# danieldugas/DeepMimic_mujoco

Measured on AMD Instinct MI355X. Metric: env-steps/sec (whole node), 34-DoF humanoid, 4096 envs, at 1/2/4/8 MI355X, higher is better.
Workload: dtype f32

## Files before the change

deepmimic_mujoco_amd/csrc/dm_abi.hip:

```cpp
#include "../../include/deepmimic_hip.h"
#include "dm_device.h"
#include "dm_topology.h"

#include <math.h>
#include <stdio.h>
#include <string.h>

#include <string>
#include <vector>

#include "dm_kernels.hip"
#include "dm_ppo.hip"
#include "dm_policy.hip"
#include "dm_ppo_mlp.hip"
#include "dm_ppo_wide.hip"
#include "dm_sac.hip"

struct DmEngine {
  DmConfig cfg;
  DmModel model;
  int N = 0;
  DmDev *dT = nullptr;
  float *dState = nullptr;
  float *dArScratch = nullptr;
  float *dClipRows[DM_MAX_CLIPS] = {nullptr};
  float *dClipReset[DM_MAX_CLIPS] = {nullptr};
  int clipL[DM_MAX_CLIPS] = {0};
  int clipFlags[DM_MAX_CLIPS] = {0};
  float *debug = nullptr;
  int32_t *dOrder = nullptr;
  int32_t *dCost = nullptr;
  static constexpr int NEV = 512;
  hipEvent_t ev0[NEV] = {}, ev1[NEV] = {};
  long nrec = 0;
  long nlaunch = 0;
  int stride = 1;
  int waves = 0;
  bool timing = false;
  float last_ms = 0;
  std::string err;
};

static int fail(DmEngine *e, int code, const char *what, hipError_t he = hipSuccess) {
  if (e) {
    e->err = what;
    if (he != hipSuccess) { e->err += ": "; e->err += hipGetErrorString(he); }
  }
  return code;
}
#define HIPCHK(e, call)                                   \
  do {                                                    \
    hipError_t _r = (call);                               \
    if (_r != hipSuccess) return fail(e, DM_EHIP, #call, _r); \
  } while (0)

extern "C" void dm_default_config(DmConfig *c) {
  memset(c, 0, sizeof(*c));
  c->num_envs = 1;
  c->max_ep_length = 1000;
  c->vel_obs_scale = 0.1f;
  c->low_z = 0.7f;
  c->high_z = 2.0f;
  c->w_pose = 0.75f; c->w_vel = 0.1f; c->w_end_eff = 0.15f; c->w_com = 0.0f; c->w_joint_limit = -0.1f;
  c->obs_bound = 100.0f;
  c->seed = 1234;
  c->auto_reset = 1;
  c->device = 0;
  c->lpt_schedule = 1;
  c->task = DM_TASK_DPENV;
  c->amnesty_steps = 150;
// ... 99 lines not shown
static int check_model(DmEngine *e, const DmModel &m) {
  if (m.nq != DM_NQ || m.nv != DM_NV || m.nu != DM_NU || m.nbody != DM_NBODY || m.ngeom != DM_NGEOM)
    return fail(e, DM_EINVAL, "model dimensions do not match the compiled-in humanoid3d dimensions");
  if (m.integrator != DM_INT_RK4 && m.integrator != DM_INT_EULER) return fail(e, DM_EINVAL, "integrator must be RK4 or Euler");
  if (m.npair < 0 || m.npair > DM_MAXPAIR) return fail(e, DM_EINVAL, "npair out of range");
  for (int b = 1; b < DM_NBODY; b++) {
    if (m.body_quat[b][0] != 1.0) return fail(e, DM_EINVAL, "kernels assume identity body quaternions");
    if (m.body_dofnum[b] != 1 && m.body_dofnum[b] != 3 && m.body_dofnum[b] != 6)
      return fail(e, DM_EINVAL, "kernels assume 1- or 3-hinge bodies under a free root");
    if (m.body_depth[b] < 1 || m.body_depth[b] > 4) return fail(e, DM_EINVAL, "tree depth > 4");
  }
  for (int j = 0; j < DM_NJNT; j++)
    for (int i = 0; i < 3; i++)
      if (m.jnt_pos[j][i] != 0.0) return fail(e, DM_EINVAL, "kernels assume joint anchors at the body origin");
  if (m.jnt_type[0] != DM_JNT_FREE || m.jnt_body[0] != 1) return fail(e, DM_EINVAL, "joint 0 must be the free root");
  for (int k = 0; k < DM_NV; k++)
    if (m.dof_parent[k] != topo::PARENT[k] || m.dof_Madr[k] != topo::MADR[k])
      return fail(e, DM_EINVAL, "dof tree differs from the compiled-in topology (regenerate csrc/dm_topology.h)");
  for (int b = 0; b < DM_NBODY; b++)
    if (m.body_parent[b] != topo::BPARENT[b])
      return fail(e, DM_EINVAL, "body tree differs from the compiled-in topology (regenerate csrc/dm_topology.h)");
  return DM_OK;
}

extern "C" int dm_create(const DmModel *model, const DmConfig *cfg, DmHandle *out) {
  if (!model || !cfg || !out || cfg->num_envs < 1) return DM_EINVAL;
  int ndev = 0;
  if (hipGetDeviceCount(&ndev) != hipSuccess || ndev <= 0) return DM_ENODEV;
  DmEngine *e = new DmEngine();
  e->cfg = *cfg;
  e->model = *model;
  e->N = cfg->num_envs;
  if (const char *w = getenv("DM_WAVES")) e->waves = atoi(w);
  int rc = check_model(e, *model);
  if (rc != DM_OK) { fprintf(stderr, "dm_create: %s\n", e->err.c_str()); delete e; return rc; }
  if (hipSetDevice(cfg->device) != hipSuccess) { delete e; return DM_ENODEV; }
  DmDev T;
  build_tables(*model, T);
  if (hipMalloc(&e->dT, sizeof(DmDev)) != hipSuccess) { delete e; return DM_ENOMEM; }
  hipMemcpy(e->dT, &T, sizeof(DmDev), hipMemcpyHostToDevice);
  size_t sb = (size_t)e->N * DMK_STATE_STRIDE * sizeof(float);
  if (hipMalloc(&e->dState, sb) != hipSuccess) { hipFree(e->dT); delete e; return DM_ENOMEM; }
  std::vector<float> init((size_t)e->N * DMK_STATE_STRIDE, 0.f);
  for (int i = 0; i < e->N; i++)
    for (int k = 0; k < DM_NQ; k++) init[(size_t)i * DMK_STATE_STRIDE + DMS_QPOS + k] = (float)model->qpos0[k];
  hipMemcpy(e->dState, init.data(), sb, hipMemcpyHostToDevice);
  if (hipMalloc(&e->dArScratch, (size_t)e->N * DMK_MAXROW * DMK_MAXROW * sizeof(float)) != hipSuccess) {
    hipFree(e->dState); hipFree(e->dT); delete e; return DM_ENOMEM;
  }
  if (hipMalloc(&e->dOrder, e->N * sizeof(int32_t)) != hipSuccess || hipMalloc(&e->dCost, e->N * sizeof(int32_t)) != hipSuccess) {
    hipFree(e->dArScratch); hipFree(e->dState); hipFree(e->dT); delete e; return DM_ENOMEM;
  }
  hipMemset(e->dCost, 0, e->N * sizeof(int32_t));
  { std::vector<int32_t> ident(e->N);
    for (int i = 0; i < e->N; i++) ident[i] = i;
    hipMemcpy(e->dOrder, ident.data(), e->N * sizeof(int32_t), hipMemcpyHostToDevice); }
  for (int i = 0; i < DmEngine::NEV; i++) { hipEventCreate(&e->ev0[i]); hipEventCreate(&e->ev1[i]); }
  *out = e;
  return DM_OK;
}

extern "C" int dm_destroy(DmHandle e) {
  if (!e) return DM_EINVAL;
  hipSetDevice(e->cfg.device);
  hipDeviceSynchronize();
  for (int i = 0; i < DM_MAX_CLIPS; i++) { if (e->dClipRows[i]) hipFree(e->dClipRows[i]); if (e->dClipReset[i]) hipFree(e->dClipReset[i]); }
// ... 87 lines not shown
  HIPCHK(e, hipSetDevice(e->cfg.device));
  hipLaunchKernelGGL(dm_get_clip_kernel, dim3((e->N + 255) / 256), dim3(256), 0, (hipStream_t)stream, e->dState, clip_ids, e->N);
  HIPCHK(e, hipGetLastError());
  return DM_OK;
}

extern "C" int dm_set_clip_flags(DmHandle e, int clip_id, int flags) {
  if (!e || clip_id < 0 || clip_id >= DM_MAX_CLIPS) return DM_EINVAL;
  e->clipFlags[clip_id] = flags;
  return DM_OK;
}

extern "C" int dm_set_env_clips(DmHandle e, const int32_t *clip_ids, void *stream) {
  if (!e) return DM_EINVAL;
  HIPCHK(e, hipSetDevice(e->cfg.device));
  hipLaunchKernelGGL(dm_set_clip_kernel, dim3((e->N + 255) / 256), dim3(256), 0, (hipStream_t)stream, e->dState, clip_ids, e->N);
  HIPCHK(e, hipGetLastError());
  return DM_OK;
}

static void fill_launch(DmEngine *e, DmLaunch &P, int mode) {
  memset(&P, 0, sizeof(P));
  P.T = e->dT;
  P.state = e->dState;
  P.ar_scratch = e->dArScratch;
  for (int i = 0; i < DM_MAX_CLIPS; i++) { P.clips[i].rows = e->dClipRows[i]; P.clips[i].reset = e->dClipReset[i]; P.clips[i].L = e->clipL[i]; P.clips[i].flags = e->clipFlags[i]; }
  P.N = e->N; P.mode = mode; P.auto_reset = e->cfg.auto_reset; P.max_ep_length = e->cfg.max_ep_length;
  P.vel_obs_scale = e->cfg.vel_obs_scale; P.low_z = e->cfg.low_z; P.high_z = e->cfg.high_z; P.obs_bound = e->cfg.obs_bound;
  P.w_pose = e->cfg.w_pose; P.w_vel = e->cfg.w_vel; P.w_ee = e->cfg.w_end_eff; P.w_com = e->cfg.w_com; P.w_jl = e->cfg.w_joint_limit;
  P.seed = e->cfg.seed;
  P.amnesty_steps = e->cfg.amnesty_steps; P.to_getup_len = e->cfg.to_getup_len;
  P.integrator = e->cfg.integrator == DM_CFG_INT_EULER ? DM_INT_EULER : e->cfg.integrator == DM_CFG_INT_RK4 ? DM_INT_RK4 : e->model.integrator;
  P.f8 = e->cfg.stale_contact_slots ? 1 : 0;
  P.debug = e->debug;
}

static int launch(DmEngine *e, DmLaunch &P, int nslots, void *stream) {
  P.nslots = nslots;
  if (e->clipL[0] < 1) return fail(e, DM_EINVAL, "no clip loaded (dm_load_clip clip 0 first)");
  if (e->cfg.task == DM_TASK_COMBINED && (e->clipL[1] < 1 || e->clipL[2] < 2))
    return fail(e, DM_EINVAL, "combined task needs clips 0,1,2 = walk, run, getup");
  HIPCHK(e, hipSetDevice(e->cfg.device));
  hipStream_t s = (hipStream_t)stream;
  const int evi = (int)(e->nrec % DmEngine::NEV);
  const bool rec = e->timing && (e->nlaunch++ % e->stride) == 0;
  if (rec) hipEventRecord(e->ev0[evi], s);
  const dim3 grid((P.nslots + DMK_ENVS_PER_BLOCK - 1) / DMK_ENVS_PER_BLOCK), block(64 * DMK_ENVS_PER_BLOCK);
  const bool three_waves = e->waves == 3 || (e->waves == 0 && P.nslots >= 3072);
  if (e->cfg.task == DM_TASK_COMBINED) {
    if (three_waves) hipLaunchKernelGGL(dm_step_combined_kernel_w3, grid, block, 0, s, P);
    else hipLaunchKernelGGL(dm_step_combined_kernel, grid, block, 0, s, P);
#ifdef DM_EXPERIMENT_W4
  } else if (e->waves == 4) {
    hipLaunchKernelGGL(dm_step_kernel_w4, grid, block, 0, s, P);
#endif
  } else if (three_waves) {
    hipLaunchKernelGGL(dm_step_kernel_w3, grid, block, 0, s, P);
  } else {
    hipLaunchKernelGGL(dm_step_kernel, grid, block, 0, s, P);
  }
  if (rec) { hipEventRecord(e->ev1[evi], s); e->nrec++; }
  HIPCHK(e, hipGetLastError());
  return DM_OK;
}

extern "C" int dm_reset(DmHandle e, const uint8_t *mask, const int32_t *idx_init, float *obs_out, void *stream) {
// ... 172 lines not shown
```

deepmimic_mujoco_amd/csrc/dm_device.h:

```cpp
#pragma once

#include <hip/hip_runtime.h>
#include <stdint.h>

#include "../../include/dm_model.h"

#define DMK_NQ DM_NQ
#define DMK_NV DM_NV
#define DMK_NU DM_NU
#define DMK_NB DM_NBODY
#define DMK_NG DM_NGEOM
#define DMK_MAXCON DM_MAXCON
#define DMK_MAXROW DM_MAXROW
#define DMK_LANEROW 64
#define DMK_REGROW 32
#define DMK_MSTRIDE 35
#define DMK_MAXANC 12
#define DMK_STATE_STRIDE 144
#define DMK_CLIP_ROW 80

struct DmPairDev {
  int16_t g1, g2;
  int8_t t1, t2, pad0, pad1;
  float margin, rbsum;
// ... 75 lines not shown
};

#define DMS_QPOS 0
#define DMS_QVEL 35
#define DMS_WARM 69
#define DMS_CTRL 103
#define DMS_IDX 131
#define DMS_EPLEN 132
#define DMS_EPREW 133
#define DMS_CLIP 134
#define DMS_RCNT 135
#define DMS_F8R 136
#define DMS_F8L 137

#define DMK_RESET_ROW 72

struct DmClipDev {
  const float *rows;
  const float *reset;
  int32_t L, flags;
};

enum { DMK_MODE_STEP = 0, DMK_MODE_FORCED = 1, DMK_MODE_RESET = 2, DMK_MODE_SETSTATE = 3,
       DMK_MODE_PHYSICS = 4 };

struct DmLaunch {
  const DmDev *T;
  float *state;
  float *ar_scratch;
  DmClipDev clips[8];
  int32_t N, nslots, mode, auto_reset, max_ep_length;
  int32_t amnesty_steps, to_getup_len;
  int32_t integrator, f8;
  float vel_obs_scale, low_z, high_z, obs_bound;
  float w_pose, w_vel, w_ee, w_com, w_jl;
  uint64_t seed;
  const float *actions;
  const float *in_qpos;
  const float *in_qvel;
  const float *in_warm;
  const float *in_ctrl;
  const int32_t *env_ids;
  int32_t *cost;
  const uint8_t *mask;
  const int32_t *idx_init;
  int32_t run_forward;
  float *obs, *rew, *terms, *terminal_obs, *debug;
  uint8_t *done;
  int32_t *reason;
};
```

deepmimic_mujoco_amd/csrc/dm_kernels.hip:

```cpp
#include "../../include/deepmimic_hip.h"
#include "dm_device.h"
#include "dm_topology.h"

#include <math.h>

#include <type_traits>

#define SYNC()                                              \
  do {                                                      \
    __builtin_amdgcn_fence(__ATOMIC_RELEASE, "wavefront");  \
    __builtin_amdgcn_wave_barrier();                        \
    __builtin_amdgcn_fence(__ATOMIC_ACQUIRE, "wavefront");  \
  } while (0)
#define DMK_ENVS_PER_BLOCK 1
#ifndef DMK_WAVES_PER_SIMD
#define DMK_WAVES_PER_SIMD 2
#endif
#ifdef DM_PROFILE
#define PROF_DECL do { if ((threadIdx.x & 63) == 0) { for (int _i = 0; _i < 16; _i++) g_S.prof[_i] = 0; for (int _i = 0; _i < 4; _i++) g_S.prof_stage[_i] = 0; g_S.prof_t = g_S.prof_t0 = __builtin_amdgcn_s_memtime(); } } while (0)
#define PROF_STAGE(i) do { if ((threadIdx.x & 63) == 0 && (i) < 4) g_S.prof_stage[i] = (unsigned)(__builtin_amdgcn_s_memtime() - g_S.prof_t0); } while (0)
#define PROF(i) do { if ((threadIdx.x & 63) == 0) { unsigned long long _t = __builtin_amdgcn_s_memtime(); g_S.prof[i] += (unsigned)(_t - g_S.prof_t); g_S.prof_t = _t; } } while (0)
#if DM_PROFILE == 2
#define PROF2(i) PROF(i)
#else
// ... 52 lines not shown
  }
};
__device__ __forceinline__ float solve_LT(float x, const float dv, const int negdep, const float *M) {
  StaticFor<0, DMK_NV - 1>::run([&](auto ic) {
    constexpr int i = DMK_NV - 1 - decltype(ic)::value;
    const float xi = rl(x * dv, i);
    const float l = lane_sel<topo::anc_mask(i)>(M[topo::MADR[i] + topo::NANC[i] + negdep], 0.f);
    x = fmaf(-l, xi, x);
    return true;
  });
  return x;
}
__device__ __forceinline__ float solve_L(float x, const float dv, const int mrow, const float *M) {
  StaticFor<0, DMK_NV - 1>::run([&](auto jc) {
    constexpr int j = decltype(jc)::value;
    const float xj = rl(x * dv, j);
    const float l = lane_sel<topo::desc_mask(j)>(M[mrow - topo::NANC[j]], 0.f);
    x = fmaf(-l, xj, x);
    return true;
  });
  return x;
}
template <int CTRL>
__device__ __forceinline__ float dpp_mov(float v) {
  return __int_as_float(__builtin_amdgcn_update_dpp(0, __float_as_int(v), CTRL, 0xF, 0xF, true));
}
__device__ __forceinline__ float wave_sum(float v) {
  v += dpp_mov<0xB1>(v);
  v += dpp_mov<0x4E>(v);
  v += dpp_mov<0x141>(v);
  v += dpp_mov<0x140>(v);
  return (rl(v, 0) + rl(v, 16)) + (rl(v, 32) + rl(v, 48));
}
__device__ __forceinline__ unsigned long long lanemask_lt(int lane) {
  return (lane == 0) ? 0ull : (~0ull >> (64 - lane));
}
__device__ __forceinline__ int prefix_count(bool flag, int lane, int *total) {
  unsigned long long m = __ballot(flag);
  *total = __popcll(m);
  return __popcll(m & lanemask_lt(lane));
}

__device__ __forceinline__ void cross3(float *r, const float *a, const float *b) {
  float x = a[1] * b[2] - a[2] * b[1], y = a[2] * b[0] - a[0] * b[2], z = a[0] * b[1] - a[1] * b[0];
  r[0] = x; r[1] = y; r[2] = z;
}
__device__ __forceinline__ float dot3(const float *a, const float *b) {
  return a[0] * b[0] + a[1] * b[1] + a[2] * b[2];
}
__device__ __forceinline__ void quat_mul(float *r, const float *a, const float *b) {
  float w = a[0] * b[0] - a[1] * b[1] - a[2] * b[2] - a[3] * b[3];
  float x = a[0] * b[1] + a[1] * b[0] + a[2] * b[3] - a[3] * b[2];
  float y = a[0] * b[2] - a[1] * b[3] + a[2] * b[0] + a[3] * b[1];
  float z = a[0] * b[3] + a[1] * b[2] - a[2] * b[1] + a[3] * b[0];
  r[0] = w; r[1] = x; r[2] = y; r[3] = z;
}
__device__ __forceinline__ void quat_rot(float *r, const float *q, const float *v) {
  float t[3], u[3];
  cross3(t, q + 1, v);
  t[0] *= 2.f; t[1] *= 2.f; t[2] *= 2.f;
  cross3(u, q + 1, t);
  r[0] = v[0] + q[0] * t[0] + u[0];
  r[1] = v[1] + q[0] * t[1] + u[1];
  r[2] = v[2] + q[0] * t[2] + u[2];
}
__device__ __forceinline__ void quat2mat(float *m, const float *q) {
// ... 888 lines not shown
      int cnt = __popc(c.valid);
      unsigned long long lt = lanemask_lt(lane);
      unsigned long long b0 = __ballot(cnt & 1), b1 = __ballot(cnt & 2), b2 = __ballot(cnt & 4);
      int off = __popcll(b0 & lt) + 2 * __popcll(b1 & lt) + 4 * __popcll(b2 & lt);
      int total = __popcll(b0) + 2 * __popcll(b1) + 4 * __popcll(b2);
      if (total == 0) continue;
      int w = base + off;
#pragma unroll
      for (int s = 0; s < 4; s++) {
        if ((c.valid >> s) & 1) {
          if (w < DMK_MAXCON) {
            float fr[9] = {c.n[s][0], c.n[s][1], c.n[s][2], c.t[0], c.t[1], c.t[2], 0, 0, 0};
            make_frame(fr);
            S.c_dist[w] = c.d[s];
            for (int q = 0; q < 3; q++) S.c_pos[w][q] = c.p[s][q];
            for (int q = 0; q < 9; q++) S.c_frame[w][q] = fr[q];
            S.c_g1[w] = g1; S.c_g2[w] = g2;
          }
          w++;
        }
      }
      base += total;
    }
    if (base > DMK_MAXCON) { overflow |= 1; base = DMK_MAXCON; }
    ncon = base;
    SYNC();

    PROF(5);
  return ncon | (overflow << 8);
}

template <bool MF>
__device__ __forceinline__ void build_row(GDev &T, EnvLds &S, const int r, const int nefc, const float (&com)[3],
                                          float (&J)[DMK_NV], float &R, float &Dd, float &aref, float &bb, float &jw) {
      float rpos = 0, rmargin = 0, rdiag = 1, mu = 0;
      int rtype = -1, full = 0;
      float wl[3] = {0, 0, 0}, wa[3] = {0, 0, 0};
      unsigned long long cm1 = 0, cm2 = 0;
      int ldof = -1;
      float lsign = 0;
      if (r < nefc) {
        int info = S.rowinfo[r];
        if (info < 0) {
          int v = -info - 1;
          ldof = v >> 1;
          lsign = (v & 1) ? -1.f : 1.f;
          rtype = 0;
          float q = S.qpos[ldof + 1];
          rpos = (v & 1) ? (T.d_hi[ldof] - q) : (q - T.d_lo[ldof]);
          rmargin = 0;
          rdiag = T.d_invw[ldof];
        } else {
          int ci = (info >> 3) & 0x3F, e = info & 7;
          full = (info & 0x4000) ? 1 : 0;
          int g1 = S.c_g1[ci], g2 = S.c_g2[ci];
          int b1 = T.g_body[g1], b2 = T.g_body[g2];
          int cd1 = T.g_condim[g1], cd2 = T.g_condim[g2];
          int dim = cd1 > cd2 ? cd1 : cd2;
          mu = fmaxf(T.g_mu[g1], T.g_mu[g2]);
          float fr[9];
          for (int i = 0; i < 9; i++) fr[i] = S.c_frame[ci][i];
          float tran = T.b_invw[b1] + T.b_invw[b2];
          if (dim < 3) {
            rtype = 1;
            wl[0] = fr[0]; wl[1] = fr[1]; wl[2] = fr[2];
            rdiag = tran;
          } else {
            rtype = 2;
            const bool second = (e >> 1) != 0;
            const float tx = second ? fr[6] : fr[3], ty = second ? fr[7] : fr[4], tz = second ? fr[8] : fr[5];
            float sg = (e & 1) ? -mu : mu;
            wl[0] = fr[0] + sg * tx; wl[1] = fr[1] + sg * ty; wl[2] = fr[2] + sg * tz;
            rdiag = tran + mu * mu * tran;
          }
          float off[3] = {S.c_pos[ci][0] - com[0], S.c_pos[ci][1] - com[1], S.c_pos[ci][2] - com[2]};
          cross3(wa, off, wl);
          cm1 = T.b_chain[b1]; cm2 = T.b_chain[b2];
          rpos = S.c_dist[ci];
          rmargin = fmaxf(T.g_margin[g1], T.g_margin[g2]);
        }
      }
      float vel = 0, jqs = 0;
      jw = 0;
      float vals[32];
      if (MF) {
        const float wv[6] = {wa[0], wa[1], wa[2], wl[0], wl[1], wl[2]};
        const int lane_ = (int)(threadIdx.x & 63);
        const float *cdp = &S.cdof[lane_ & 31][lane_ >> 5];
        mfma_f16v acc;
#pragma unroll
        for (int v = 0; v < 16; v++) acc[v] = 0.f;
#pragma unroll
        for (int p = 0; p < 3; p++) {
          const auto sw = __builtin_amdgcn_permlane32_swap(__float_as_uint(wv[2 * p]), __float_as_uint(wv[2 * p + 1]), false, false);
          acc = __builtin_amdgcn_mfma_f32_32x32x2f32(cdp[2 * p], __uint_as_float(sw[0]), acc, 0, 0, 0);
        }
#pragma unroll
        for (int v = 0; v < 16; v++) {
          const auto sw = __builtin_amdgcn_permlane32_swap(__float_as_uint(acc[v]), __float_as_uint(acc[v]), false, false);
          vals[(v / 4) * 8 + (v % 4)] = acc[v];
          vals[(v / 4) * 8 + (v % 4) + 4] = __uint_as_float(sw[1]);
        }
      }
#pragma unroll
      for (int k = 0; k < DMK_NV; k++) {
        float val;
        if (MF && k < 32) {
          val = vals[k];
        } else {
          const float4 ca = *reinterpret_cast<const float4 *>(&S.cdof[k][0]);
          const float2 cb = *reinterpret_cast<const float2 *>(&S.cdof[k][4]);
          val = ca.x * wa[0] + ca.y * wa[1] + ca.z * wa[2] + ca.w * wl[0] + cb.x * wl[1] + cb.y * wl[2];
        }
        float sg = (float)((int)((cm2 >> k) & 1ull) - (int)((cm1 >> k) & 1ull));
        float j = (k == ldof) ? lsign : sg * val;
        J[k] = j;
        vel += j * S.qvel[k];
        jqs += j * S.qacc_smooth[k];
        jw += j * S.warm[k];
      }
      R = 1; Dd = 0; aref = 0; bb = 0;
      if (r < nefc) {
        float sol[5] = {T.solimp[0], T.solimp[1], T.solimp[2], T.solimp[3], T.solimp[4]};
        float imp = impedance(sol, rpos, rmargin);
        R = fmaxf(MINVALF, (1 - imp) * rdiag / imp);
        if (rtype == 2 && full) R = 2 * mu * mu * R;
        aref = -T.B * vel - T.K * imp * (rpos - rmargin);
        bb = jqs - aref;
        Dd = 1.0f / R;
      }
      {
        lds_cfloat_p Mp = (lds_cfloat_p)S.M;
#pragma unroll
        for (int i = DMK_NV - 1; i >= 1; i--) {
          const float xi = J[i] * S.dinv[i];
          asm volatile("" : "+v"(Mp), "+v"(J[0]));
#pragma unroll
          for (int j = 0; j < i; j++)
            if (topo::is_anc(j, i)) J[j] -= Mp[topo::midx(i, j)] * xi;
        }
      }
#pragma unroll
      for (int k = 0; k < DMK_NV; k++) J[k] *= S.dsqrtinv[k];
}

__device__ __noinline__ float fwd_constraint_wide(GDev &T, const int lane, const int nefc, const float xs, const float dv,
                                                  float *ar) {
  EnvLds &S = g_S;
  const int lk = lane < DMK_NV ? lane : 0;
  const float com[3] = {S.com[0], S.com[1], S.com[2]};
  float Ja[DMK_NV], Jb[DMK_NV];
  float Ra, Da, arefa, bba, jwa, Rb, Db, arefb, bbb, jwb;
  build_row<false>(T, S, lane, nefc, com, Ja, Ra, Da, arefa, bba, jwa);
  build_row<false>(T, S, lane + 64, nefc, com, Jb, Rb, Db, arefb, bbb, jwb);
  float ARda = Ra, ARdb = Rb;
#pragma unroll
  for (int k = 0; k < DMK_NV; k++) { ARda += Ja[k] * Ja[k]; ARdb += Jb[k] * Jb[k]; }
  const bool va = lane < nefc, vb = lane + 64 < nefc;
#pragma unroll 1
  for (int i = 0; i < nefc; i++) {
    const int src = i & 63;
    float acca = 0, accb = 0;
    if (i < 64) {
#pragma unroll
      for (int k = 0; k < DMK_NV; k++) { const float bi = rl(Ja[k], src); acca = fmaf(Ja[k], bi, acca); accb = fmaf(Jb[k], bi, accb); }
      if (lane == src) acca += Ra;
    } else {
#pragma unroll
      for (int k = 0; k < DMK_NV; k++) { const float bi = rl(Jb[k], src); acca = fmaf(Ja[k], bi, acca); accb = fmaf(Jb[k], bi, accb); }
      if (lane == src) accb += Rb;
    }
    ar[i * 128 + lane] = acca;
    ar[i * 128 + 64 + lane] = accb;
  }
  const float ARinva = va ? 1.0f / ARda : 0.f, ARinvb = vb ? 1.0f / ARdb : 0.f;
  float fa = 0, fb = 0, ra = bba, rb = bbb;
  {
    const float jara = jwa - arefa, jarb = jwb - arefb;
    const float fwa = (va && jara < 0) ? -Da * jara : 0.f, fwb = (vb && jarb < 0) ? -Db * jarb : 0.f;
    float rwa = bba, rwb = bbb;
#pragma unroll 1
    for (int i = 0; i < nefc; i++) {
      const float fi = (i < 64) ? rl(fwa, i & 63) : rl(fwb, i & 63);
      rwa = fmaf(ar[i * 128 + lane], fi, rwa);
      rwb = fmaf(ar[i * 128 + 64 + lane], fi, rwb);
    }
    const float cost = wave_sum(fwa * (0.5f * (rwa - bba) + bba) + fwb * (0.5f * (rwb - bbb) + bbb));
// ... 16 lines not shown
      rb = fmaf(cb, dli, rb);
    }
#pragma unroll 1
    for (int i = 64; i < nefc; i++) {
      const float ca = na, cb = nb;
      if (i + 1 < nefc) { na = ar[(i + 1) * 128 + lane]; nb = ar[(i + 1) * 128 + 64 + lane]; }
      const float dli = rl(fmaxf(nfb, -rb * ARinvb), i - 64);
      rsb = (lane == i - 64) ? rb : rsb;
      ra = fmaf(ca, dli, ra);
      rb = fmaf(cb, dli, rb);
    }
    const float dla = fmaxf(nfa, -rsa * ARinva), dlb = fmaxf(nfb, -rsb * ARinvb);
    const float impv = -wave_sum(dla * fmaf(0.5f * dla, ARda, rsa) + dlb * fmaf(0.5f * dlb, ARdb, rsb));
    fa += dla;
    fb += dlb;
    iter++;
    if (impv * scale < tol) break;
  }
  if (lane == 0) S.info[3] = iter;
  float v = 0;
#pragma unroll
  for (int k = 0; k < DMK_NV; k++) {
    const float sm = wave_sum(fa * Ja[k] + fb * Jb[k]);
    if (lane == k) v = sm;
  }
  const int mrow = T.d_madr[lk] + T.d_nanc[lk];
  const uint64_t ancm = T.d_ancm[lk];
  v *= S.dsqrtinv[lk] * S.M[T.d_madr[lk]];
  v = solve_L(v, dv, (lane < DMK_NV) ? mrow : DMK_MAXANC, g_S.M);
  return xs + v * dv;
}

__device__ __forceinline__ float fwd_constraint(GDev &T, const int lane, const int ncon, int overflow, float *dbg_force,
                                                float *ar_scratch) {
  EnvLds &S = g_S;
  int nefc = 0, nlimit = 0, solver_iter = 0;
  const int lb = lane < DMK_NB ? lane : 0;
  const int lk = lane < DMK_NV ? lane : 0;
  const int lg = lane < DMK_NG ? lane : 0;
  const int bdep = (lane < DMK_NB) ? T.b_depth[lb] : -1;
  const float bmass = (lane < DMK_NB) ? T.b_mass[lb] : 0.f;
  const float mtot_inv = T.total_mass_inv;
  (void)lg; (void)bdep; (void)bmass; (void)mtot_inv; (void)lb; (void)lk;
  const float xs = (lane < DMK_NV) ? S.qacc_smooth[lk] : 0.f;
  const float dv = (lane < DMK_NV) ? S.dinv[lk] : 0.f;
  const float com[3] = {S.com[0], S.com[1], S.com[2]};
  float qacc_out;
    {
      bool lim = false;
      float ldist = 0;
      int lneg = 0;
      if (lane >= 6 && lane < DMK_NV && dlimited) {
        float q = S.qpos[lane + 1];
        if (q < dlo) { lim = true; ldist = q - dlo; lneg = 0; }
        else if (q > dhi) { lim = true; ldist = dhi - q; lneg = 1; }
      }
      int myrow = prefix_count(lim, lane, &nlimit);
      if (lim) { S.rowinfo[myrow] = (int16_t)(-(((lane << 1) | lneg) + 1)); }
      int dim3 = 0, have = lane < ncon;
      if (have) {
        int cd1 = T.g_condim[S.c_g1[lane]], cd2 = T.g_condim[S.c_g2[lane]];
        dim3 = (cd1 > cd2 ? cd1 : cd2) >= 3;
      }
      unsigned long long lt = lanemask_lt(lane);
      unsigned long long m1 = __ballot(have && !dim3), m4 = __ballot(have && dim3);
      int roff = nlimit + __popcll(m1 & lt) + 4 * __popcll(m4 & lt);
      int rtot = nlimit + __popcll(m1) + 4 * __popcll(m4);
      if (have) {
        int nr = dim3 ? 4 : 1;
        for (int e = 0; e < nr; e++)
          if (roff + e < DMK_MAXROW) S.rowinfo[roff + e] = (int16_t)((lane << 3) | e | (((roff + nr) <= DMK_MAXROW) ? 0x4000 : 0));
      }
      if (rtot > DMK_MAXROW) { overflow |= 2; rtot = DMK_MAXROW; }
      nefc = rtot;
    }
    SYNC();

    qacc_out = xs;
    solver_iter = 0;
    if (nefc > DMK_LANEROW) {
      qacc_out = fwd_constraint_wide(T, lane, nefc, xs, dv, ar_scratch);
      solver_iter = S.info[3];
    } else if (nefc > 0) {
      float J[DMK_NV];
      float R, Dd, aref, bb, jw;
      if (nefc <= DMK_REGROW) build_row<true>(T, S, lane, nefc, com, J, R, Dd, aref, bb, jw);
      else build_row<false>(T, S, lane, nefc, com, J, R, Dd, aref, bb, jw);
      PROF(6);
      float AR[DMK_REGROW];
      float *arx = ar_scratch + lane;
      float ARd = R;
#pragma unroll
      for (int k = 0; k < DMK_NV; k++) ARd += J[k] * J[k];
      if (nefc <= DMK_REGROW && nefc >= DMK_MFMA_MIN_ROWS) {
        mfma_f16v acc;
#pragma unroll
        for (int v = 0; v < 16; v++) acc[v] = 0.f;
        StaticFor<0, DMK_NV / 2>::run([&](auto kc) {
          constexpr int k0 = decltype(kc)::value * 2;
          const auto sw = __builtin_amdgcn_permlane32_swap(__float_as_uint(J[k0]), __float_as_uint(J[k0 + 1]), false, false);
          const float x = __uint_as_float(sw[0]);
          acc = __builtin_amdgcn_mfma_f32_32x32x2f32(x, x, acc, 0, 0, 0);
          return true;
        });
        StaticFor<0, 16>::run([&](auto vc) {
          constexpr int v = decltype(vc)::value;
          const auto sw = __builtin_amdgcn_permlane32_swap(__float_as_uint(acc[v]), __float_as_uint(acc[v]), false, false);
          constexpr int i0 = (v / 4) * 8 + (v % 4);
          AR[i0] = lane_sel<(1ull << i0)>(acc[v] + R, acc[v]);
          const float up = __uint_as_float(sw[1]);
          AR[i0 + 4] = lane_sel<(1ull << (i0 + 4))>(up + R, up);
          return true;
        });
      } else
      StaticFor<0, DMK_REGROW>::run([&](auto ic) {
        constexpr int i = decltype(ic)::value;
        if (i >= nefc) {
          if ((i & 3) == 0) return false;
          AR[i] = 0.f;
          return true;
        }
        float acc0 = 0, acc1 = 0;
#pragma unroll
        for (int k = 0; k < DMK_NV; k += 2) {
          acc0 = fmaf(J[k], rl(J[k], i), acc0);
          acc1 = fmaf(J[k + 1], rl(J[k + 1], i), acc1);
        }
        float acc = acc0 + acc1;
        if (lane == i) acc += R;
        AR[i] = acc;
        return true;
      });
#pragma unroll 1
      for (int i = DMK_REGROW; i < nefc; i++) {
        float acc0 = 0, acc1 = 0;
#pragma unroll
        for (int k = 0; k < DMK_NV; k += 2) {
          acc0 = fmaf(J[k], rl(J[k], i), acc0);
          acc1 = fmaf(J[k + 1], rl(J[k + 1], i), acc1);
        }
        float acc = acc0 + acc1;
        if (lane == i) acc += R;
        arx[(i - DMK_REGROW) * 64] = acc;
      }
      const float ARinv = (lane < nefc) ? 1.0f / ARd : 0.f;
      PROF(7);
      float f = 0, r = bb;
      {
        float jar = jw - aref;
        float fw = (lane < nefc && jar < 0) ? -Dd * jar : 0.f;
        float rw = bb;
        StaticFor<0, DMK_REGROW>::run([&](auto ic) {
          constexpr int i = decltype(ic)::value;
          if (i >= nefc) return false;
          rw += AR[i] * rl(fw, i);
          return true;
        });
#pragma unroll 1
        for (int i = DMK_REGROW; i < nefc; i++) rw += arx[(i - DMK_REGROW) * 64] * rl(fw, i);
        float cost = wave_sum(fw * (0.5f * (rw - bb) + bb));
        if (!(cost > 0)) { f = fw; r = rw; }
      }
      const float scale = T.pgs_scale, tol = T.tolerance;
      const int max_iter = T.iterations;
      const float nAinv = -ARinv;
      float g = r * nAinv;
      StaticFor<0, DMK_REGROW / 4>::run([&](auto bc) {
        constexpr int b = decltype(bc)::value * 4;
        if (b >= nefc) return false;
        AR[b] *= nAinv; AR[b + 1] *= nAinv; AR[b + 2] *= nAinv; AR[b + 3] *= nAinv;
        return true;
      });
      int iter = 0;
// ... 12 lines not shown
            g = fmaf(AR[i], dli, g);
          };
          step(std::integral_constant<int, b>{});
          step(std::integral_constant<int, b + 1>{});
          step(std::integral_constant<int, b + 2>{});
          step(std::integral_constant<int, b + 3>{});
          return true;
        });
        if (nefc > DMK_REGROW) {
          float anext = arx[0];
#pragma unroll 1
          for (int i = DMK_REGROW; i < nefc; i++) {
            const float acur = anext * nAinv;
            if (i + 1 < nefc) anext = arx[(i + 1 - DMK_REGROW) * 64];
            const float dli = rl(fmaxf(nf, g), i);
            gs = (lane_s == i) ? g : gs;
            g = fmaf(acur, dli, g);
          }
        }
        const float dl = fmaxf(nf, gs);
        const float impv = -wave_sum(dl * ARd * (0.5f * dl - gs));
        f += dl;
        iter++;
        if (impv * scale < tol) break;
      }
      solver_iter = iter;
      PROF(8);
      float v = 0;
      {
        const bool actv = (lane < nefc) && (f != 0.f);
        int nact;
        const int slot = prefix_count(actv, lane, &nact);
        if (nact <= 20) {
          if (actv) {
#pragma unroll
            for (int k = 0; k < DMK_NV; k++) S.u.fin.tr[slot][k] = f * J[k];
          }
          SYNC();
          if (lane < DMK_NV)
            for (int a = 0; a < nact; a++) v += S.u.fin.tr[a][lk];
          SYNC();
        } else {
#pragma unroll
          for (int k = 0; k < DMK_NV; k++) {
            float s = wave_sum(f * J[k]);
            if (lane == k) v = s;
          }
        }
      }
      const int mrow = T.d_madr[lk] + T.d_nanc[lk];
      const uint64_t ancm = T.d_ancm[lk];
      v *= S.dsqrtinv[lk] * S.M[T.d_madr[lk]];
      v = solve_L(v, dv, (lane < DMK_NV) ? mrow : DMK_MAXANC, g_S.M);
      qacc_out = xs + v * dv;
#ifndef DM_PROFILE
      if (dbg_force && lane < DMK_LANEROW) dbg_force[lane] = (lane < nefc) ? f : 0.f;
#endif
    }
    SYNC();
    if (lane < DMK_NV) { S.qacc[lk] = qacc_out; S.warm[lk] = qacc_out; }
    SYNC();
    PROF(9);
  if (lane == 0) { S.info[0] = ncon; S.info[1] = nefc; S.info[2] = nlimit; S.info[3] = solver_iter; S.info[4] = overflow; }
  return qacc_out;
}

template <int TASK>
__device__ __forceinline__ void step_body(const DmLaunch &P) {
  constexpr int NOBS_T = TASK ? DM_NOBS_COMBINED : DM_NOBS;
  constexpr int NOBS_B = NOBS_T - 64;
  constexpr int NTERMS = TASK ? 8 : 5;
  GDev &T = *(GDev *)P.T;
  const int lane = threadIdx.x & 63;
  EnvLds &S = g_S;
  const int slot = blockIdx.x;
  if (slot >= P.nslots) return;
  const int env = P.env_ids ? P.env_ids[slot] : slot;
// ... 82 lines not shown
    return;
  }
  if (mode == DMK_MODE_STEP || mode == DMK_MODE_FORCED || mode == DMK_MODE_PHYSICS) {
    float a = (lane < DMK_NQ) ? S.qpos[lane] : 0.f, b = (lane < DMK_NV) ? S.qvel[lk] : 0.f;
    sim_err = __any(!(fabsf(a) <= MAXVALF) || !(fabsf(b) <= MAXVALF));
  }

  PROF(0);
  for (;;) {
   float qacc_out = 0;
   if (!sim_err) {
    GDev *Tp = (GDev *)P.T;
    asm volatile("" : "+s"(Tp));
    GDev &Ts = *Tp;
#ifndef DM_NO_LANE_LAUNDER
    int lane_st = lane;
    asm volatile("" : "+v"(lane_st));
#else
    const int lane_st = lane;
#endif
    fwd_smooth(Ts, lane_st);
    if (it == 0) {
      if (lane < DMK_NV) {
        const float v0 = S.qvel[lk];
        S.rk[0][lk] = (lane < 3) ? S.qpos[lane] : ((lane >= 6) ? S.qpos[lane + 1] : 0.f);
        S.rk[1][lk] = v0; S.rk[2][lk] = 0.f; S.rk[3][lk] = 0.f; S.rk[4][lk] = v0;
      }
      if (lane < 4) S.rkq[lane] = S.qpos[3 + lane];
    }
    {
      const int cr = fwd_collide(Ts, lane_st);
      ncon = cr & 0xFF;
      qacc_out = fwd_constraint(Ts, lane_st, ncon, cr >> 8, P.debug ? P.debug + (size_t)env * DM_DEBUG_STRIDE + 352 : nullptr,
                                P.ar_scratch + (size_t)env * DMK_MAXROW * DMK_MAXROW);
      nefc = S.info[1]; nlimit = S.info[2]; solver_iter = S.info[3]; overflow = S.info[4];
      if (it < 4) { stage_ncon |= (unsigned)(ncon & 0xFF) << (8 * it); stage_nefc |= (unsigned)(nefc & 0xFF) << (8 * it); }
      work = (work >> 1) + 64 + (nefc > 0 ? 48 + 16 * nefc : 0) + nefc * solver_iter;
      if (P.f8) {
        bool rfs = false, lfs = false;
        if (lane < ncon) {
          const int g1 = S.c_g1[lane], g2 = S.c_g2[lane];
          const bool fl = (g1 == Ts.floor_geom || g2 == Ts.floor_geom);
          rfs = fl && (g1 == Ts.rfoot_geom || g2 == Ts.rfoot_geom);
          lfs = fl && (g1 == Ts.lfoot_geom || g2 == Ts.lfoot_geom);
        }
        const unsigned keep = ncon >= 32 ? 0u : (~0u << ncon);
        f8r = (f8r & keep) | (unsigned)__ballot(rfs);
        f8l = (f8l & keep) | (unsigned)__ballot(lfs);
      }
    }
    if (it == 0 || (it == 4 && mode == DMK_MODE_FORCED && !after_reset)) {
      bool badv = (lane < DMK_NV) && !(fabsf(qacc_out) <= MAXVALF);
      sim_err = __any(badv);
    }
   }

    const bool euler = (P.integrator == DM_INT_EULER) && (mode == DMK_MODE_STEP || mode == DMK_MODE_PHYSICS);
    float x0q = 0, x0v = 0, accq = 0, accv = 0, curv = 0;
    float q0[4] = {1, 0, 0, 0};
    if (!sim_err && it < 4) {
      const bool dl = lane < DMK_NV;
      x0q = dl ? S.rk[0][lk] : 0.f; x0v = dl ? S.rk[1][lk] : 0.f; accq = dl ? S.rk[2][lk] : 0.f;
      accv = dl ? S.rk[3][lk] : 0.f; curv = dl ? S.rk[4][lk] : 0.f;
      for (int i = 0; i < 4; i++) q0[i] = S.rkq[i];
    }
    if (!sim_err && it < 3 && !euler) {
      const float Bw = (it == 0) ? (1.f / 6.f) : (1.f / 3.f);
// ... 307 lines not shown
```

Measured before the change: 13.72 million.

## Skip zero Jacobian columns using wave-wide DOF sparsity masks in constraint rows

Each constraint row now computes a support mask of the DOFs it can touch (the chain XOR for contacts, a single DOF for limits), OR-reduced across the wave with DPP. The mask gates Jacobian construction, the L^T solve, the diagonal and AR products (per limb or pair group, including the MFMA steps), and the final force scatter, so work on columns that are zero in every row is skipped. Dense behaviour stays available through the DM_DENSE_ROWS environment variable. The cost is extra wave reductions and branches. Limb groupings are hardcoded to the humanoid DOF tree and protected by a static_assert.

```diff
diff --git a/deepmimic_mujoco_amd/csrc/dm_abi.hip b/deepmimic_mujoco_amd/csrc/dm_abi.hip
--- a/deepmimic_mujoco_amd/csrc/dm_abi.hip
+++ b/deepmimic_mujoco_amd/csrc/dm_abi.hip
@@ -36,6 +36,7 @@
   long nlaunch = 0;
   int stride = 1;
   int waves = 0;
+  int dense_rows = 0;
   bool timing = false;
   float last_ms = 0;
   std::string err;
@@ -201,6 +202,7 @@
   e->model = *model;
   e->N = cfg->num_envs;
   if (const char *w = getenv("DM_WAVES")) e->waves = atoi(w);
+  if (const char *d = getenv("DM_DENSE_ROWS")) e->dense_rows = atoi(d) != 0;
   int rc = check_model(e, *model);
   if (rc != DM_OK) { fprintf(stderr, "dm_create: %s\n", e->err.c_str()); delete e; return rc; }
   if (hipSetDevice(cfg->device) != hipSuccess) { delete e; return DM_ENODEV; }
@@ -354,6 +356,7 @@
   P.amnesty_steps = e->cfg.amnesty_steps; P.to_getup_len = e->cfg.to_getup_len;
   P.integrator = e->cfg.integrator == DM_CFG_INT_EULER ? DM_INT_EULER : e->cfg.integrator == DM_CFG_INT_RK4 ? DM_INT_RK4 : e->model.integrator;
   P.f8 = e->cfg.stale_contact_slots ? 1 : 0;
+  P.dense_rows = e->dense_rows;
   P.debug = e->debug;
 }
 
diff --git a/deepmimic_mujoco_amd/csrc/dm_device.h b/deepmimic_mujoco_amd/csrc/dm_device.h
--- a/deepmimic_mujoco_amd/csrc/dm_device.h
+++ b/deepmimic_mujoco_amd/csrc/dm_device.h
@@ -131,6 +131,7 @@
   int32_t N, nslots, mode, auto_reset, max_ep_length;
   int32_t amnesty_steps, to_getup_len;
   int32_t integrator, f8;
+  int32_t dense_rows;
   float vel_obs_scale, low_z, high_z, obs_bound;
   float w_pose, w_vel, w_ee, w_com, w_jl;
   uint64_t seed;
diff --git a/deepmimic_mujoco_amd/csrc/dm_kernels.hip b/deepmimic_mujoco_amd/csrc/dm_kernels.hip
--- a/deepmimic_mujoco_amd/csrc/dm_kernels.hip
+++ b/deepmimic_mujoco_amd/csrc/dm_kernels.hip
@@ -108,6 +108,28 @@
   v += dpp_mov<0x140>(v);
   return (rl(v, 0) + rl(v, 16)) + (rl(v, 32) + rl(v, 48));
 }
+__device__ __forceinline__ unsigned wave_or(unsigned v) {
+  v |= (unsigned)__builtin_amdgcn_update_dpp(0, (int)v, 0xB1, 0xF, 0xF, true);
+  v |= (unsigned)__builtin_amdgcn_update_dpp(0, (int)v, 0x4E, 0xF, 0xF, true);
+  v |= (unsigned)__builtin_amdgcn_update_dpp(0, (int)v, 0x141, 0xF, 0xF, true);
+  v |= (unsigned)__builtin_amdgcn_update_dpp(0, (int)v, 0x140, 0xF, 0xF, true);
+  return (unsigned)(__builtin_amdgcn_readlane((int)v, 0) | __builtin_amdgcn_readlane((int)v, 16)) |
+         (unsigned)(__builtin_amdgcn_readlane((int)v, 32) | __builtin_amdgcn_readlane((int)v, 48));
+}
+struct DofMask {
+  unsigned lo, hi;
+  __device__ __forceinline__ bool bit(const int k) const { return k < 32 ? ((lo >> k) & 1u) != 0 : ((hi >> (k - 32)) & 1u) != 0; }
+  __device__ __forceinline__ bool any(const unsigned long long m) const {
+    const unsigned ml = (unsigned)m, mh = (unsigned)(m >> 32);
+    return (ml && (lo & ml)) || (mh && (hi & mh));
+  }
+};
+constexpr int LIMB_LO[8] = {0, 6, 9, 12, 16, 20, 27, 34};
+constexpr unsigned long long limb_mask(int l) { return ((1ull << LIMB_LO[l + 1]) - 1) & ~((1ull << LIMB_LO[l]) - 1); }
+constexpr int PAIRGRP_LO[7] = {0, 6, 12, 16, 20, 28, 34};
+constexpr unsigned long long pairgrp_mask(int g) { return ((1ull << PAIRGRP_LO[g + 1]) - 1) & ~((1ull << PAIRGRP_LO[g]) - 1); }
+static_assert(DMK_NV == 34 && topo::PARENT[12] == 8 && topo::PARENT[16] == 8 && topo::PARENT[20] == 5 && topo::PARENT[27] == 5,
+              "limb boundaries follow the humanoid3d dof tree");
 __device__ __forceinline__ unsigned long long lanemask_lt(int lane) {
   return (lane == 0) ? 0ull : (~0ull >> (64 - lane));
 }
@@ -1062,7 +1084,8 @@
 
 template <bool MF>
 __device__ __forceinline__ void build_row(GDev &T, EnvLds &S, const int r, const int nefc, const float (&com)[3],
-                                          float (&J)[DMK_NV], float &R, float &Dd, float &aref, float &bb, float &jw) {
+                                          float (&J)[DMK_NV], float &R, float &Dd, float &aref, float &bb, float &jw,
+                                          const bool dense, DofMask &cmask_out) {
       float rpos = 0, rmargin = 0, rdiag = 1, mu = 0;
       int rtype = -1, full = 0;
       float wl[3] = {0, 0, 0}, wa[3] = {0, 0, 0};
@@ -1110,6 +1133,16 @@
           rmargin = fmaxf(T.g_margin[g1], T.g_margin[g2]);
         }
       }
+      DofMask umask = {~0u, ~0u}, cmask = {~0u, ~0u};
+      if (!dense) {
+        unsigned long long sup = cm1 ^ cm2, clo = cm1 | cm2;
+        if (ldof >= 0) { sup = 1ull << ldof; clo = T.d_ancm[ldof] | sup; }
+        const unsigned ulo = wave_or((unsigned)sup), clow = wave_or((unsigned)clo);
+        const unsigned hi = wave_or((unsigned)(sup >> 32) | ((unsigned)(clo >> 32) << 2));
+        umask.lo = ulo; umask.hi = hi & 3u;
+        cmask.lo = clow; cmask.hi = (hi >> 2) & 3u;
+      }
+      cmask_out = cmask;
       float vel = 0, jqs = 0;
       jw = 0;
       float vals[32];
@@ -1118,8 +1151,10 @@
         const int lane_ = (int)(threadIdx.x & 63);
         const float *cdp = &S.cdof[lane_ & 31][lane_ >> 5];
         mfma_f16v acc;
-#pragma unroll
-        for (int v = 0; v < 16; v++) acc[v] = 0.f;
+        float zero = 0.f;
+        asm volatile("" : "+v"(zero));
+#pragma unroll
+        for (int v = 0; v < 16; v++) acc[v] = zero;
 #pragma unroll
         for (int p = 0; p < 3; p++) {
           const auto sw = __builtin_amdgcn_permlane32_swap(__float_as_uint(wv[2 * p]), __float_as_uint(wv[2 * p + 1]), false, false);
@@ -1134,20 +1169,24 @@
       }
 #pragma unroll
       for (int k = 0; k < DMK_NV; k++) {
-        float val;
-        if (MF && k < 32) {
-          val = vals[k];
-        } else {
-          const float4 ca = *reinterpret_cast<const float4 *>(&S.cdof[k][0]);
-          const float2 cb = *reinterpret_cast<const float2 *>(&S.cdof[k][4]);
-          val = ca.x * wa[0] + ca.y * wa[1] + ca.z * wa[2] + ca.w * wl[0] + cb.x * wl[1] + cb.y * wl[2];
-        }
-        float sg = (float)((int)((cm2 >> k) & 1ull) - (int)((cm1 >> k) & 1ull));
-        float j = (k == ldof) ? lsign : sg * val;
+        float j = 0.f;
+        if (umask.bit(k)) {
+          asm volatile("");
+          float val;
+          if (MF && k < 32) {
+            val = vals[k];
+          } else {
+            const float4 ca = *reinterpret_cast<const float4 *>(&S.cdof[k][0]);
+            const float2 cb = *reinterpret_cast<const float2 *>(&S.cdof[k][4]);
+            val = ca.x * wa[0] + ca.y * wa[1] + ca.z * wa[2] + ca.w * wl[0] + cb.x * wl[1] + cb.y * wl[2];
+          }
+          float sg = (float)((int)((cm2 >> k) & 1ull) - (int)((cm1 >> k) & 1ull));
+          j = (k == ldof) ? lsign : sg * val;
+          vel += j * S.qvel[k];
+          jqs += j * S.qacc_smooth[k];
+          jw += j * S.warm[k];
+        }
         J[k] = j;
-        vel += j * S.qvel[k];
-        jqs += j * S.qacc_smooth[k];
-        jw += j * S.warm[k];
       }
       R = 1; Dd = 0; aref = 0; bb = 0;
       if (r < nefc) {
@@ -1163,15 +1202,16 @@
         lds_cfloat_p Mp = (lds_cfloat_p)S.M;
 #pragma unroll
         for (int i = DMK_NV - 1; i >= 1; i--) {
+          if (!cmask.bit(i)) continue;
           const float xi = J[i] * S.dinv[i];
           asm volatile("" : "+v"(Mp), "+v"(J[0]));
 #pragma unroll
           for (int j = 0; j < i; j++)
             if (topo::is_anc(j, i)) J[j] -= Mp[topo::midx(i, j)] * xi;
-        }
-      }
-#pragma unroll
-      for (int k = 0; k < DMK_NV; k++) J[k] *= S.dsqrtinv[k];
+          J[i] *= S.dsqrtinv[i];
+        }
+      }
+      J[0] *= S.dsqrtinv[0];
 }
 
 __device__ __noinline__ float fwd_constraint_wide(GDev &T, const int lane, const int nefc, const float xs, const float dv,
@@ -1181,8 +1221,9 @@
   const float com[3] = {S.com[0], S.com[1], S.com[2]};
   float Ja[DMK_NV], Jb[DMK_NV];
   float Ra, Da, arefa, bba, jwa, Rb, Db, arefb, bbb, jwb;
-  build_row<false>(T, S, lane, nefc, com, Ja, Ra, Da, arefa, bba, jwa);
-  build_row<false>(T, S, lane + 64, nefc, com, Jb, Rb, Db, arefb, bbb, jwb);
+  DofMask cmw;
+  build_row<false>(T, S, lane, nefc, com, Ja, Ra, Da, arefa, bba, jwa, true, cmw);
+  build_row<false>(T, S, lane + 64, nefc, com, Jb, Rb, Db, arefb, bbb, jwb, true, cmw);
   float ARda = Ra, ARdb = Rb;
 #pragma unroll
   for (int k = 0; k < DMK_NV; k++) { ARda += Ja[k] * Ja[k]; ARdb += Jb[k] * Jb[k]; }
@@ -1265,7 +1306,7 @@
 }
 
 __device__ __forceinline__ float fwd_constraint(GDev &T, const int lane, const int ncon, int overflow, float *dbg_force,
-                                                float *ar_scratch) {
+                                                float *ar_scratch, const bool dense) {
   EnvLds &S = g_S;
   int nefc = 0, nlimit = 0, solver_iter = 0;
   const int lb = lane < DMK_NB ? lane : 0;
@@ -1317,23 +1358,34 @@
     } else if (nefc > 0) {
       float J[DMK_NV];
       float R, Dd, aref, bb, jw;
-      if (nefc <= DMK_REGROW) build_row<true>(T, S, lane, nefc, com, J, R, Dd, aref, bb, jw);
-      else build_row<false>(T, S, lane, nefc, com, J, R, Dd, aref, bb, jw);
+      DofMask cmask;
+      if (nefc <= DMK_REGROW) build_row<true>(T, S, lane, nefc, com, J, R, Dd, aref, bb, jw, dense, cmask);
+      else build_row<false>(T, S, lane, nefc, com, J, R, Dd, aref, bb, jw, dense, cmask);
       PROF(6);
       float AR[DMK_REGROW];
       float *arx = ar_scratch + lane;
       float ARd = R;
-#pragma unroll
-      for (int k = 0; k < DMK_NV; k++) ARd += J[k] * J[k];
+      StaticFor<0, 7>::run([&](auto lc) {
+        constexpr int l = decltype(lc)::value;
+        if (cmask.any(limb_mask(l))) {
+#pragma unroll
+          for (int k = LIMB_LO[l]; k < LIMB_LO[l + 1]; k++) ARd += J[k] * J[k];
+        }
+        return true;
+      });
       if (nefc <= DMK_REGROW && nefc >= DMK_MFMA_MIN_ROWS) {
         mfma_f16v acc;
-#pragma unroll
-        for (int v = 0; v < 16; v++) acc[v] = 0.f;
+        float zero = 0.f;
+        asm volatile("" : "+v"(zero));
+#pragma unroll
+        for (int v = 0; v < 16; v++) acc[v] = zero;
         StaticFor<0, DMK_NV / 2>::run([&](auto kc) {
           constexpr int k0 = decltype(kc)::value * 2;
-          const auto sw = __builtin_amdgcn_permlane32_swap(__float_as_uint(J[k0]), __float_as_uint(J[k0 + 1]), false, false);
-          const float x = __uint_as_float(sw[0]);
-          acc = __builtin_amdgcn_mfma_f32_32x32x2f32(x, x, acc, 0, 0, 0);
+          if (cmask.any(3ull << k0)) {
+            const auto sw = __builtin_amdgcn_permlane32_swap(__float_as_uint(J[k0]), __float_as_uint(J[k0 + 1]), false, false);
+            const float x = __uint_as_float(sw[0]);
+            acc = __builtin_amdgcn_mfma_f32_32x32x2f32(x, x, acc, 0, 0, 0);
+          }
           return true;
         });
         StaticFor<0, 16>::run([&](auto vc) {
@@ -1354,11 +1406,17 @@
           return true;
         }
         float acc0 = 0, acc1 = 0;
-#pragma unroll
-        for (int k = 0; k < DMK_NV; k += 2) {
-          acc0 = fmaf(J[k], rl(J[k], i), acc0);
-          acc1 = fmaf(J[k + 1], rl(J[k + 1], i), acc1);
-        }
+        StaticFor<0, 6>::run([&](auto gc) {
+          constexpr int g_ = decltype(gc)::value;
+          if (cmask.any(pairgrp_mask(g_))) {
+#pragma unroll
+            for (int k = PAIRGRP_LO[g_]; k < PAIRGRP_LO[g_ + 1]; k += 2) {
+              acc0 = fmaf(J[k], rl(J[k], i), acc0);
+              acc1 = fmaf(J[k + 1], rl(J[k + 1], i), acc1);
+            }
+          }
+          return true;
+        });
         float acc = acc0 + acc1;
         if (lane == i) acc += R;
         AR[i] = acc;
@@ -1367,11 +1425,17 @@
 #pragma unroll 1
       for (int i = DMK_REGROW; i < nefc; i++) {
         float acc0 = 0, acc1 = 0;
-#pragma unroll
-        for (int k = 0; k < DMK_NV; k += 2) {
-          acc0 = fmaf(J[k], rl(J[k], i), acc0);
-          acc1 = fmaf(J[k + 1], rl(J[k + 1], i), acc1);
-        }
+        StaticFor<0, 6>::run([&](auto gc) {
+          constexpr int g_ = decltype(gc)::value;
+          if (cmask.any(pairgrp_mask(g_))) {
+#pragma unroll
+            for (int k = PAIRGRP_LO[g_]; k < PAIRGRP_LO[g_ + 1]; k += 2) {
+              acc0 = fmaf(J[k], rl(J[k], i), acc0);
+              acc1 = fmaf(J[k + 1], rl(J[k + 1], i), acc1);
+            }
+          }
+          return true;
+        });
         float acc = acc0 + acc1;
         if (lane == i) acc += R;
         arx[(i - DMK_REGROW) * 64] = acc;
@@ -1450,17 +1514,24 @@
         int nact;
         const int slot = prefix_count(actv, lane, &nact);
         if (nact <= 20) {
-          if (actv) {
-#pragma unroll
-            for (int k = 0; k < DMK_NV; k++) S.u.fin.tr[slot][k] = f * J[k];
-          }
+          StaticFor<0, 7>::run([&](auto lc) {
+            constexpr int l = decltype(lc)::value;
+            if (cmask.any(limb_mask(l))) {
+              if (actv) {
+#pragma unroll
+                for (int k = LIMB_LO[l]; k < LIMB_LO[l + 1]; k++) g_S.u.fin.tr[slot][k] = f * J[k];
+              }
+            }
+            return true;
+          });
           SYNC();
-          if (lane < DMK_NV)
+          if (lane < DMK_NV && ((((unsigned long long)cmask.hi << 32 | cmask.lo) >> lk) & 1ull))
             for (int a = 0; a < nact; a++) v += S.u.fin.tr[a][lk];
           SYNC();
         } else {
 #pragma unroll
           for (int k = 0; k < DMK_NV; k++) {
+            if (!cmask.bit(k)) continue;
             float s = wave_sum(f * J[k]);
             if (lane == k) v = s;
           }
@@ -1609,7 +1680,7 @@
       const int cr = fwd_collide(Ts, lane_st);
       ncon = cr & 0xFF;
       qacc_out = fwd_constraint(Ts, lane_st, ncon, cr >> 8, P.debug ? P.debug + (size_t)env * DM_DEBUG_STRIDE + 352 : nullptr,
-                                P.ar_scratch + (size_t)env * DMK_MAXROW * DMK_MAXROW);
+                                P.ar_scratch + (size_t)env * DMK_MAXROW * DMK_MAXROW, P.dense_rows != 0);
       nefc = S.info[1]; nlimit = S.info[2]; solver_iter = S.info[3]; overflow = S.info[4];
       if (it < 4) { stage_ncon |= (unsigned)(ncon & 0xFF) << (8 * it); stage_nefc |= (unsigned)(nefc & 0xFF) << (8 * it); }
       work = (work >> 1) + 64 + (nefc > 0 ? 48 + 16 * nefc : 0) + nefc * solver_iter;
diff --git a/deepmimic_mujoco_amd/row_sparsity.py b/deepmimic_mujoco_amd/row_sparsity.py
--- /dev/null
+++ b/deepmimic_mujoco_amd/row_sparsity.py
@@ -0,0 +1,59 @@
+import numpy as np
+
+
+def chain_tables(model):
+    nb, nv = len(model.body_parent), len(model.dof_parent)
+    b_chain = []
+    for b in range(nb):
+        chain, a = 0, b
+        while a > 0:
+            for k in range(int(model.body_dofnum[a])):
+                chain |= 1 << (int(model.body_dofadr[a]) + k)
+            a = int(model.body_parent[a])
+        b_chain.append(chain)
+    d_ancm = []
+    for k in range(nv):
+        m, a = 0, int(model.dof_parent[k])
+        while a >= 0:
+            m |= 1 << a
+            a = int(model.dof_parent[a])
+        d_ancm.append(m)
+    return b_chain, d_ancm
+
+
+def limit_rows(model, qpos):
+    out = []
+    for k in range(6, len(model.dof_parent)):
+        j = int(model.dof_jnt[k])
+        if not model.jnt_limited[j]:
+            continue
+        q = qpos[k + 1]
+        if q < model.jnt_range[j][0] or q > model.jnt_range[j][1]:
+            out.append(k)
+    return out
+
+
+def row_masks(model, tables, qpos, contacts, nefc):
+    b_chain, d_ancm = tables
+    rows = [(1 << k, d_ancm[k] | (1 << k)) for k in limit_rows(model, qpos)]
+    for c in contacts:
+        c1 = b_chain[int(model.geom_body[int(c[13])])]
+        c2 = b_chain[int(model.geom_body[int(c[14])])]
+        rows += [(c1 ^ c2, c1 | c2)] * (4 if int(c[15]) >= 3 else 1)
+    return rows if len(rows) == nefc else None
+
+
+def mask_bits(mask, nv):
+    return np.array([(mask >> k) & 1 for k in range(nv)], bool)
+
+
+def solve_LT_rows(model, qLD, J):
+    X = np.array(J, np.float64, copy=True)
+    nv = X.shape[1]
+    for i in range(nv - 1, 0, -1):
+        adr, j = int(model.dof_Madr[i]) + 1, int(model.dof_parent[i])
+        while j >= 0:
+            X[:, j] -= qLD[adr] * X[:, i]
+            adr += 1
+            j = int(model.dof_parent[j])
+    return X
```

Measured after the change: 12.93 million. -5.7%, worse.
